# jkaardal/pyipm

Hardware: AMD Instinct MI355X
Metric: newton_steps_per_sec (higher is better)
Workload: dtype f64

## Files before the change

### pyipm_amd/csrc/ctx.hpp

```cpp
#pragma once
#include <hip/hip_runtime.h>
#include <stdint.h>
#include <stdio.h>
#include <stdlib.h>
#include <string.h>
#include <string>
#include <new>
#include <stdexcept>
#include <map>
#include <memory>
#include <vector>
#include "../../include/pyipm_newton.h"
#include "owned.hpp"
#include "step_plan.hpp"

namespace pyipm {

constexpr int TB = PYIPM_TILE;
static_assert(TB == PLAN_TB, "step_plan.hpp states the tile on its own");
constexpr int PADG = PYIPM_PAD;
constexpr int BM = 128;
constexpr int BKU = 16;
constexpr int ROWCHUNK = 2048;

// ... 135 lines not shown
    void factor_timed_out() { factored = false; }
    void factor_returned(int rc, bool keep_forward) {
        if (rc) zeros_clean = false;
        forward_pending = (rc == 0 || rc == PYIPM_E_NONFINITE) && keep_forward && forward_fused;
    }
    void solved(bool direction, bool ray_survives) {
        ev_solve_valid = true; have_direction = direction;
        if (!ray_survives) ray_valid = false;
    }
    void ray_formed() { ray_valid = true; }
    void ray_dropped() { ray_valid = false; }
    void rc_warm_cold() { rc_warm_valid[0] = rc_warm_valid[1] = false; }
    void rc_warm_kept(int phase, bool good) { rc_warm_valid[phase] = good; }
    void storage_handed_out() { zeros_clean = false; storage_exported = true; px_valid = false; }
    void keep_zeros_set() { zeros_clean = false; storage_exported = false; }
    void quiesced() { factored = false; forward_pending = false; forward_fused = false; zeros_clean = false; px_valid = false; }
};

constexpr unsigned long long POLL_TIMEOUT = 200000000ull;
struct PollWords {
    DevBuf<unsigned> buf;
    size_t words; const char* message;
    bool used = false;
    PollWords(size_t words_, const char* message_) : words(words_), message(message_) {}
    unsigned* err() const { return buf + words; }
    hipError_t allocate() { return buf.reserve(words + 1); }
    hipError_t ensure(hipStream_t st) {
        if (buf) return hipSuccess;
        const hipError_t e = allocate();
        return e != hipSuccess ? e : clear_err(st);
    }
    hipError_t arm(size_t n, hipStream_t st) { return hipMemsetAsync(buf, 0, n * sizeof(unsigned), st); }
    hipError_t zero_and_wait(size_t n) {
        const hipError_t e = hipMemset(buf, 0, n * sizeof(unsigned));
        return e != hipSuccess ? e : hipDeviceSynchronize();
    }
    hipError_t fetch_err(int* host, hipStream_t st) const { return hipMemcpyAsync(host, err(), sizeof(int), hipMemcpyDeviceToHost, st); }
    hipError_t clear_err(hipStream_t st) { return hipMemsetAsync(err(), 0, sizeof(unsigned), st); }
};

struct DistState;
struct DistDelete { void operator()(DistState*) const; };

struct Ctx {
    Geo g;
    int batch = 1;
    bool batched = false;
    int64_t b_sH = 0, b_sJe = 0, b_sJi = 0;
    double *b_mu = nullptr, *b_delta = nullptr, *b_delta_c = nullptr, *b_in = nullptr, *b_alpha = nullptr;
    int *b_act = nullptr, *b_in_act = nullptr;
    DevBuf<double> b_merit_buf;
    DevBuf<double> b_solve_buf;
    DevBuf<int> b_form;
    bool b_any_cond = false;
    int device = 0;
    hipStream_t stream = nullptr;
    Stream side;
    Event ev_head, ev_panel, ev_fwd;
    Stream fwd;
    std::vector<Event> ev_done;
    int fuse_forward = 1;
    int lookahead = 2;
    Event ev_early;
    struct TileList { unsigned* dev = nullptr; unsigned count = 0;
                      Event ready; hipStream_t on = nullptr; bool seen_done = false; };
    struct TlArena { DevBuf<unsigned> dev; PinnedBuf<unsigned> host{hipHostMallocDefault}; size_t used = 0; };
    std::vector<TlArena> tl_arenas;
    std::map<std::vector<int64_t>, TileList> tile_lists;
    int skip_zeros = 1;
    int group = 1;
    bool tail_group_user = false;
    int tail_group = 4;
    GroupSched sched;
    double* Wnext = nullptr;
    int group_chain = 1;
    Stream rest;
    std::vector<Event> ev_band;
    Event ev_join, ev_main, ev_split, ev_sfast;
    int keep_zeros = 1;
    int tile_step = 1;
    int sweep_max_blocks = 0;
    int occ_fwd_sweep = 0, occ_bwd_sweep = 0, occ_fwd_prefix = 0, occ_fwd_range = 0;
    int sweep_persist = 1;
    DevBuf<double> sweep_buf;
    DevBuf<double> ms_buf;
    PollWords sweep_words{3 * 4096,
                          "backward sweep (k_bwd_sweep): a poll timed out in an earlier solve; its result was NaN"};
    int dist_slices = 2;
    double dist_timeout_s = 300.0;
    int dist_comm2 = 0;
    int wide_sub = 256;
    int reserve_cus = 16;
    int64_t persist_rows = 12288;
    int num_cus = 256;
    int bulk_bn = 256;
    unsigned long long* dbg_buf = nullptr;
    int condensed = 0;
    int cond_min_refine = 0;
    Geo gc;
    double cond_sigma_max = 1.0e4;
    int64_t cond_na = 0;
    int *cond_pos = nullptr, *cond_idx = nullptr, *cond_cnt = nullptr;
    DevBuf<int> cond_store;
    DevBuf<double> Jx;
    DevBuf<double> JT; double* WT = nullptr;
    double *vc = nullptr, *vt = nullptr;
    double* fwd_vec = nullptr;
    double t_gram = 0;
    bool provider_only = false;
    int reuse_x = 1;
    DevBuf<double> snap;
    int reuse_lam_e = 1;
    DevBuf<double> snap_e;
    DevBuf<unsigned> diag_tiles;
    std::vector<unsigned> diag_tiles_host; int64_t diag_tiles_n = -1;
    int64_t n_reused = 0, n_recorded = 0;
    int fwd_prefix = 1;
    int fwd_prefix_wgs = 96;
    PollWords fwdp_words{4096 + 8192,
                         "forward sweep over the kept panels (k_fwd_prefix): a poll timed out; the direction was NaN "
                         "(PYIPM_FWD_PREFIX=0 runs it panel by panel)"};
    int fwd_range = 1;
    int fwd_range_wgs = 32;
    int64_t fwd_range_key[8] = {-1, -1, -1, -1, -1, -1, -1, -1}, fwd_range_owned = 0;
    PollWords fwdr_words{4096 + 8192,
                         "forward sweep over the kept slack and lambda_e panels (k_fwd_range): a poll timed out; the direction was NaN "
                         "(PYIPM_FWD_RANGE=0 runs it panel by panel)"};
    int slack_one = 1;
    int last_step_kind = 0;
    DevBuf<char> ws;
    double *A = nullptr, *Wbuf = nullptr, *Lbuf = nullptr, *Dinv = nullptr;
    double *Tsv = nullptr;
    double *Tflag = nullptr;
    double *rhs = nullptr, *v0 = nullptr, *v1 = nullptr, *v2 = nullptr, *partial = nullptr;
    double *v3 = nullptr;
    double *df = nullptr, *ce = nullptr, *ci = nullptr, *s = nullptr, *lda = nullptr;
    DevStats* dstats = nullptr;
    unsigned long long* anorm = nullptr;
    const double *d2L = nullptr, *Je = nullptr, *Ji = nullptr;
    int64_t ld_d2L = 0, ld_Je = 0, ld_Ji = 0;
    int sharded = 0;
    std::unique_ptr<DistState, DistDelete> dist;
    DevBuf<double> stg_d2L, stg_Je, stg_Ji;
    double mu = 0.2, eps = 2.220446049250313e-16;
    double delta = 0.0, delta_c = 0.0;
    Held held;
    DevBuf<double> merit_buf, ray_buf;
    const double* ray_for = nullptr; bool ray_quad_given = false;
    int info_steps = 0, info_converged = 0;
    double info_berr0 = -1.0, info_berr = -1.0;
    int rcond_its[2] = {0, 0};
    DevBuf<double> rc_warm_buf;
    double* rc_warm[2] = {nullptr, nullptr};
    double refine_target = 1.0e-14;
    int refine_max = 8;
    double pivtol_rel = 1e-14;
    bool tile_blocked_user = false;
    int tile_blocked = 1;
    int tile_waves = 8;
    int tile_chain = 1;
    int chain_whole = 1;
    int chain_lds_kb = 100;
    bool chain_lds_set = false;
    int chain_cpy = 5;
    static constexpr int CHAIN_SLOTS = 8, CHAIN_WORDS = 160;
    PollWords chain_words{CHAIN_SLOTS * CHAIN_WORDS,
// ... 81 lines not shown
```

### pyipm_amd/csrc/kernels_solve.hpp

```cpp
#pragma once
#include "ctx.hpp"
#include "fwd_range_plan.hpp"

namespace pyipm {

__global__ void k_fwd_diag(const double* __restrict__ A, int64_t ld, int64_t lc0, int64_t c0,
                           int nbw, double* __restrict__ v, int64_t vstride)
{
    extern __shared__ double y[];
    const int tid = threadIdx.x;
    v += (int64_t)blockIdx.y * vstride;
    y[tid] = v[c0 + tid];
    const int nt = nbw / TB;
    for (int u = 0; u + 1 < nt; ++u) {
        __syncthreads();
        if (tid >= (u + 1) * TB) {
            const double* col = A + (c0 + tid) + (lc0 + (int64_t)u * TB) * ld;
            double acc = 0.0;
            #pragma unroll 8
            for (int k = 0; k < TB; ++k) acc = fma(col[(int64_t)k * ld], y[u * TB + k], acc);
            y[tid] -= acc;
        }
    }
    __syncthreads();
    v[c0 + tid] = y[tid];
}

__global__ __launch_bounds__(256) void k_fwd_gemv(const double* __restrict__ A, int64_t ld, int64_t lc0,
                                                  int64_t c0, int nbw, int64_t row_begin, int64_t Npad,
                                                  double* __restrict__ v, int64_t vstride,
                                                  int64_t a0, int64_t a1, int64_t b0, int64_t b1)
{
    extern __shared__ double y[];
    {
        const int64_t i0 = row_begin + (int64_t)blockIdx.x * 256, i1 = i0 + 256;
        if (!((i1 > a0 && i0 < a1) || (i1 > b0 && i0 < b1))) return;
    }
    v += (int64_t)blockIdx.y * vstride;
    for (int k = threadIdx.x; k < nbw; k += 256) y[k] = v[c0 + k];
    __syncthreads();
    const int64_t i = row_begin + (int64_t)blockIdx.x * 256 + threadIdx.x;
    if (i >= Npad) return;
    const double* row = A + i + lc0 * ld;
    double acc0 = 0.0, acc1 = 0.0, acc2 = 0.0, acc3 = 0.0;
    #pragma unroll 4
    for (int k = 0; k < nbw; k += 4) {
        acc0 = fma(row[(int64_t)(k + 0) * ld], y[k + 0], acc0);
        acc1 = fma(row[(int64_t)(k + 1) * ld], y[k + 1], acc1);
        acc2 = fma(row[(int64_t)(k + 2) * ld], y[k + 2], acc2);
        acc3 = fma(row[(int64_t)(k + 3) * ld], y[k + 3], acc3);
    }
    v[i] -= (acc0 + acc1) + (acc2 + acc3);
}

__global__ __launch_bounds__(64) void k_diag_apply(const double* __restrict__ Dinv, const double* __restrict__ Tsave,
                                                   const double* __restrict__ Tflag, int nref, int64_t tile0,
                                                   int64_t c0, double* __restrict__ v, int64_t vstride)
{
    __shared__ double y[TB];
    __shared__ double w[TB];
    const int lane = threadIdx.x;
    v += (int64_t)blockIdx.y * vstride;
    const int64_t base = c0 + (int64_t)blockIdx.x * TB;
    const double y0 = v[base + lane];
    y[lane] = y0;
    __syncthreads();
    const double* X = Dinv + (tile0 + blockIdx.x) * (int64_t)(TB * TB);
    const double* T = Tsave + (tile0 + blockIdx.x) * (int64_t)(TB * TB);
    double z = 0.0;
    #pragma unroll 8
    for (int j = 0; j < TB; ++j) z = fma(X[j * TB + lane], y[j], z);
    if (Tflag[tile0 + blockIdx.x] == 0.0) nref = 0;
    for (int it = 0; it < nref; ++it) {
        w[lane] = z;
        __syncthreads();
        double r = y0;
        #pragma unroll 8
        for (int j = 0; j < TB; ++j) r = fma(-T[j * TB + lane], w[j], r);
        __syncthreads();
        w[lane] = r;
        __syncthreads();
        #pragma unroll 8
        for (int j = 0; j < TB; ++j) z = fma(X[j * TB + lane], w[j], z);
        __syncthreads();
    }
// ... 75 lines not shown
    v[c0 + tid] = x[tid];
}

__global__ __launch_bounds__(1024) void k_bwd_diag4(const double* __restrict__ A, int64_t ld, int64_t lc0, int64_t c0,
                                                    int nbw, int nb, const double* __restrict__ part, int nchunk,
                                                    double* __restrict__ v, int64_t vstride, int64_t pstride)
{
    __shared__ double Ls[3][TB][TB + 1];
    __shared__ double x[4 * TB], ps[4][4 * TB];
    const int tid = threadIdx.x, k = tid & 255, q = tid >> 8;
    v += (int64_t)blockIdx.y * vstride;
    part += (int64_t)blockIdx.y * pstride;
    const int nt = nbw / TB;
    double lt[6][4];
    {
        int idx = 0;
        #pragma unroll
        for (int u = 1; u <= 3; ++u)
            #pragma unroll
            for (int t = 0; t < u; ++t, ++idx)
                #pragma unroll
                for (int r = 0; r < 4; ++r) {
                    const int e = tid + 1024 * r;
                    lt[idx][r] = (u < nt) ? A[(c0 + (int64_t)u * TB + (e & 63)) + (lc0 + t * TB + (e >> 6)) * ld] : 0.0;
                }
    }
    {
        double t = 0.0;
        if (k < nbw) for (int c = q; c < nchunk; c += 4) t += part[(int64_t)c * nb + k];
        ps[q][k] = t;
    }
    __syncthreads();
    if (tid < nbw) x[tid] = v[c0 + tid] - ((ps[0][tid] + ps[1][tid]) + (ps[2][tid] + ps[3][tid]));
    #pragma unroll
    for (int u = 3; u >= 1; --u) {
        if (u < nt) {
            const int base = u * (u - 1) / 2;
            #pragma unroll
            for (int t = 0; t < 3; ++t)
                if (t < u) {
                    #pragma unroll
                    for (int r = 0; r < 4; ++r) { const int e = tid + 1024 * r; Ls[t][e & 63][e >> 6] = lt[base + t][r]; }
                }
            __syncthreads();
            double acc = 0.0;
            if (k < u * TB) {
                const int t = k >> 6, j = k & 63;
                #pragma unroll
                for (int i = 0; i < 16; ++i) acc = fma(Ls[t][16 * q + i][j], x[u * TB + 16 * q + i], acc);
            }
            ps[q][k] = acc;
            __syncthreads();
            if (tid < u * TB) x[tid] -= (ps[0][tid] + ps[1][tid]) + (ps[2][tid] + ps[3][tid]);
        }
    }
    __syncthreads();
    if (tid < nbw) v[c0 + tid] = x[tid];
}


struct SweepGeo {
    int64_t Npad, ld, n, mi, me;
    int nb, npanels, skip;
};
__device__ __forceinline__ double ld_agent(const double* p) { return __hip_atomic_load(p, __ATOMIC_RELAXED, __HIP_MEMORY_SCOPE_AGENT); }
__device__ __forceinline__ void st_agent(double* p, double v) { __hip_atomic_store(p, v, __ATOMIC_RELAXED, __HIP_MEMORY_SCOPE_AGENT); }
__device__ __forceinline__ bool sweep_active(const SweepGeo& sg, int64_t cA, int64_t cB, int64_t r0, int64_t r1) {
    if (!sg.skip || sg.mi == 0) return true;
    const int64_t s0 = sg.n, s1 = sg.n + sg.mi, i0 = sg.n + sg.mi + sg.me;
    if (cB <= s0) return (r0 < s0) || (r1 > s1);
    if (cA >= s0 && cB <= s1) return r1 > i0 + (cA - s0) && r0 < i0 + (cB - s0);
    return true;
}
__device__ __forceinline__ bool sweep_wait(const unsigned* p, unsigned want, unsigned* err, unsigned long long timeout) {
    if (__hip_atomic_load(p, __ATOMIC_RELAXED, __HIP_MEMORY_SCOPE_AGENT) >= want) return true;
    const unsigned long long t0 = wall_clock64();
    for (;;) {
        if (__hip_atomic_load(p, __ATOMIC_RELAXED, __HIP_MEMORY_SCOPE_AGENT) >= want) return true;
        if (__hip_atomic_load(err, __ATOMIC_RELAXED, __HIP_MEMORY_SCOPE_AGENT) != 0u) return false;
        if ((unsigned long long)wall_clock64() - t0 > timeout) { __hip_atomic_store(err, 1u, __ATOMIC_RELAXED, __HIP_MEMORY_SCOPE_AGENT); return false; }
    }
}

__global__ __launch_bounds__(1024) void k_bwd_sweep(const double* __restrict__ A, SweepGeo sg, double* v, unsigned* sync,
                                                    unsigned* err, unsigned long long timeout,
                                                    double* nearbuf,
                                                    unsigned long long* dbg)
{
    __shared__ double Ls[3][TB][TB + 1];
    __shared__ double x[4 * TB], ps[4][4 * TB];
    __shared__ int ok_s;
    const int tid = threadIdx.x, lane = tid & 63, wave = tid >> 6;
    const int P = sg.npanels, nb = sg.nb;
    unsigned* flag = sync; unsigned* nearc = sync + P; unsigned* prog = sync + 2 * P;
    const int gpp = nb / 8;
    if (blockIdx.x == 0) {
        const int k = tid & 255, q = tid >> 8;
        if (tid == 0) ok_s = 1;
        __syncthreads();
        for (int s = P - 1; s >= 0; --s) {
            const int64_t c0 = (int64_t)s * nb;
            int64_t w64 = sg.Npad - c0; if (w64 > nb) w64 = nb;
            const int nbw = (int)w64, nt = nbw / TB;
            double lt[6][4];
            {
                int idx = 0;
                #pragma unroll
                for (int u = 1; u <= 3; ++u)
                    #pragma unroll
                    for (int t = 0; t < u; ++t, ++idx)
                        #pragma unroll
                        for (int r = 0; r < 4; ++r) {
                            const int e = tid + 1024 * r;
                            lt[idx][r] = (u < nt) ? A[(c0 + (int64_t)u * TB + (e & 63)) + (c0 + t * TB + (e >> 6)) * sg.ld] : 0.0;
                        }
            }
            if (dbg && tid == 0) dbg[4 * s + 0] = wall_clock64();
            if (tid < nbw) {
                const double yv = ld_agent(v + c0 + tid);
                double nv = 0.0;
                if (s + 1 < P) {
                    const unsigned long long t0 = wall_clock64();
                    for (;;) {
                        nv = ld_agent(nearbuf + c0 + tid);
                        if (nv == nv) break;
                        if (__hip_atomic_load(nearc + s + 1, __ATOMIC_RELAXED, __HIP_MEMORY_SCOPE_AGENT) >= (unsigned)gpp) { nv = ld_agent(nearbuf + c0 + tid); break; }
                        if (__hip_atomic_load(err, __ATOMIC_RELAXED, __HIP_MEMORY_SCOPE_AGENT) != 0u) { ok_s = 0; break; }
                        if ((unsigned long long)wall_clock64() - t0 > timeout) { __hip_atomic_store(err, 1u, __ATOMIC_RELAXED, __HIP_MEMORY_SCOPE_AGENT); ok_s = 0; break; }
                    }
                }
                x[tid] = yv - nv;
            }
            __syncthreads();
            if (!ok_s) break;
            if (dbg && tid == 0) dbg[4 * s + 1] = wall_clock64();
            #pragma unroll
            for (int u = 3; u >= 1; --u) {
                if (u < nt) {
                    const int base = u * (u - 1) / 2;
                    #pragma unroll
                    for (int t = 0; t < 3; ++t)
                        if (t < u) {
                            #pragma unroll
                            for (int r = 0; r < 4; ++r) { const int e = tid + 1024 * r; Ls[t][e & 63][e >> 6] = lt[base + t][r]; }
                        }
                    __syncthreads();
                    double acc = 0.0;
                    if (k < u * TB) {
                        const int t = k >> 6, j = k & 63;
                        #pragma unroll
                        for (int i = 0; i < 16; ++i) acc = fma(Ls[t][16 * q + i][j], x[u * TB + 16 * q + i], acc);
                    }
                    ps[q][k] = acc;
                    __syncthreads();
                    if (tid < u * TB) x[tid] -= (ps[0][tid] + ps[1][tid]) + (ps[2][tid] + ps[3][tid]);
                }
            }
            __syncthreads();
            if (dbg && tid == 0) dbg[4 * s + 2] = wall_clock64();
            if (tid < nbw) st_agent(v + c0 + tid, x[tid]);
            asm volatile("s_waitcnt vmcnt(0)" ::: "memory");
            __syncthreads();
            if (dbg && tid == 0) dbg[4 * s + 3] = wall_clock64();
            if (tid == 0) __hip_atomic_store(flag + s, 1u, __ATOMIC_RELAXED, __HIP_MEMORY_SCOPE_AGENT);
            if (s + 1 < P && s >= 1 && tid < gpp) {
                const int nwv_o = ((int)gridDim.x - 1 - (gpp + 15) / 16) * 16;
                if (!sweep_wait(prog + ((s - 1) * gpp + tid) % nwv_o, (unsigned)(P - (s + 1)), err, timeout)) ok_s = 0;
            }
            __syncthreads();
            if (!ok_s) break;
        }
        __syncthreads();
        if (__hip_atomic_load(err, __ATOMIC_RELAXED, __HIP_MEMORY_SCOPE_AGENT) != 0u)
            for (int64_t i = tid; i < sg.Npad; i += 1024) st_agent(v + i, __builtin_nan(""));
        return;
    }
    const int nearb_ = (gpp + 15) / 16;
    const bool specialist_ = (int)blockIdx.x <= nearb_;
    const int gw_ = ((int)blockIdx.x - 1 - nearb_) * 16 + wave;
    auto publish = [&](unsigned steps_done) {
        if (lane == 0 && !specialist_) __hip_atomic_store(prog + gw_, steps_done, __ATOMIC_RELAXED, __HIP_MEMORY_SCOPE_AGENT);
    };
    const int nearb = (gpp + 15) / 16;
    const bool specialist = (int)blockIdx.x <= nearb;
    const int nwv = specialist ? 1 : ((int)gridDim.x - 1 - nearb) * 16;
    const int gw = specialist ? ((int)blockIdx.x - 1) * 16 + wave : ((int)blockIdx.x - 1 - nearb) * 16 + wave;
    if (specialist) {
        publish((unsigned)P);
        if (gw >= gpp) return;
    }
    typedef double d2_t __attribute__((ext_vector_type(2)));
    for (int t = P - 1; t >= 1; --t) {
        const int64_t r0 = (int64_t)t * nb;
        int64_t w64 = sg.Npad - r0; if (w64 > nb) w64 = nb;
        const int nbw = (int)w64;
        const int glim = t * gpp;
        if (!specialist && gw >= glim - gpp) break;
        int kmax = specialist ? 0 : (glim - gpp - 1 - gw) / nwv;
        const bool in_rows = 4 * lane < nbw;
        bool have_x = false;
        double xr[4] = {0.0, 0.0, 0.0, 0.0};
        for (int kk = kmax; kk >= 0; --kk) {
            const int g = specialist ? glim - gpp + gw : gw + kk * nwv;
            const int64_t j0 = (int64_t)g * 8;
            const int64_t cp = (j0 / nb) * nb;
            const bool nearg = specialist;
            const bool act = sweep_active(sg, cp, cp + nb, r0, r0 + nbw);
            d2_t la[8][2];
            if (act) {
                #pragma unroll
                for (int c = 0; c < 8; ++c) {
                    if (in_rows) {
                        const double* src = A + (r0 + 4 * lane) + (j0 + c) * sg.ld;
                        la[c][0] = *reinterpret_cast<const d2_t*>(src);
                        la[c][1] = *reinterpret_cast<const d2_t*>(src + 2);
                    } else { la[c][0] = d2_t{0.0, 0.0}; la[c][1] = d2_t{0.0, 0.0}; }
                }
            }
            if (!have_x) {
                if (!sweep_wait(flag + t, 1u, err, timeout)) { publish((unsigned)P); return; }
                asm volatile("" ::: "memory");
                if (in_rows) {
                    const d2_t x01 = *reinterpret_cast<const d2_t*>(v + r0 + 4 * lane), x23 = *reinterpret_cast<const d2_t*>(v + r0 + 4 * lane + 2);
                    xr[0] = x01.x; xr[1] = x01.y; xr[2] = x23.x; xr[3] = x23.y;
                }
                have_x = true;
            }
            if (act) {
                double a[8];
                #pragma unroll
                for (int c = 0; c < 8; ++c)
                    a[c] = fma(la[c][1].y, xr[3], fma(la[c][1].x, xr[2], fma(la[c][0].y, xr[1], la[c][0].x * xr[0])));
                double b4[4], b2[2];
                const bool h5 = (lane & 32) != 0, h4 = (lane & 16) != 0, h3 = (lane & 8) != 0;
                #pragma unroll
                for (int i = 0; i < 4; ++i) {
                    const double send = h5 ? a[i] : a[i + 4], keep = h5 ? a[i + 4] : a[i];
                    b4[i] = keep + __shfl_xor(send, 32, 64);
                }
                #pragma unroll
                for (int i = 0; i < 2; ++i) {
                    const double send = h4 ? b4[i] : b4[i + 2], keep = h4 ? b4[i + 2] : b4[i];
                    b2[i] = keep + __shfl_xor(send, 16, 64);
                }
                double r;
                { const double send = h3 ? b2[0] : b2[1], keep = h3 ? b2[1] : b2[0]; r = keep + __shfl_xor(send, 8, 64); }
                r += __shfl_xor(r, 4, 64); r += __shfl_xor(r, 2, 64); r += __shfl_xor(r, 1, 64);
                if ((lane & 7) == 0) {
                    const int c = (h5 ? 4 : 0) + (h4 ? 2 : 0) + (h3 ? 1 : 0);
                    if (nearg) st_agent(nearbuf + j0 + c, r);
                    else { double* yp = v + j0 + c; st_agent(yp, ld_agent(yp) - r); }
                }
                asm volatile("s_waitcnt vmcnt(0)" ::: "memory");
            } else if (nearg && lane < 8) {
                st_agent(nearbuf + j0 + lane, 0.0);
                asm volatile("s_waitcnt vmcnt(0)" ::: "memory");
            }
            if (nearg && lane == 0) __hip_atomic_fetch_add(nearc + t, 1u, __ATOMIC_RELAXED, __HIP_MEMORY_SCOPE_AGENT);
        }
        if (!specialist) publish((unsigned)(P - t));
    }
    if (!specialist) publish((unsigned)P);
}

__global__ __launch_bounds__(512, 4) void k_fwd_sweep(const double* __restrict__ A, SweepGeo sg, double* v, unsigned* sync,
                                                      unsigned* err, unsigned long long timeout)
{
    __shared__ double xs[4 * TB];
    __shared__ double ps[8][TB];
    __shared__ int ok_s;
    const int tid = threadIdx.x, lane = tid & 63, wave = __builtin_amdgcn_readfirstlane(tid >> 6);
    const int P = sg.npanels, nb = sg.nb;
    unsigned* flag = sync; unsigned* prog = sync + P;
    const int cpp = nb / TB;
    const int nchunks = (int)(sg.Npad / TB);
    if (tid == 0) ok_s = 1;
    __syncthreads();
    if (blockIdx.x == 0) {
        for (int s = 0; s < P; ++s) {
            const int64_t c0 = (int64_t)s * nb;
            int64_t w64 = sg.Npad - c0; if (w64 > nb) w64 = nb;
            const int nbw = (int)w64, nt = nbw / TB;
            double lt[6][8];
            {
                int idx = 0;
                #pragma unroll
                for (int u = 1; u <= 3; ++u)
                    #pragma unroll
                    for (int t = 0; t < u; ++t, ++idx)
                        #pragma unroll
                        for (int r = 0; r < 8; ++r)
                            lt[idx][r] = (u < nt) ? A[(c0 + (int64_t)u * TB + lane) + (c0 + t * TB + wave + 8 * r) * sg.ld] : 0.0;
            }
            if (s > 0 && tid < nt && !sweep_wait(prog + (int)(c0 / TB) + tid, (unsigned)s, err, timeout)) ok_s = 0;
            __syncthreads();
            if (!ok_s) break;
            if (tid < nbw) xs[tid] = ld_agent(v + c0 + tid);
            __syncthreads();
            #pragma unroll
            for (int u = 1; u <= 3; ++u) {
                if (u < nt) {
                    const int base = u * (u - 1) / 2;
                    double acc = 0.0;
                    #pragma unroll
                    for (int t = 0; t < 3; ++t)
                        if (t < u) {
                            #pragma unroll
                            for (int r = 0; r < 8; ++r) acc = fma(lt[base + t][r], xs[t * TB + wave + 8 * r], acc);
                        }
                    ps[wave][lane] = acc;
                    __syncthreads();
                    if (tid < TB) {
                        double t8 = ((ps[0][tid] + ps[1][tid]) + (ps[2][tid] + ps[3][tid])) + ((ps[4][tid] + ps[5][tid]) + (ps[6][tid] + ps[7][tid]));
                        xs[u * TB + tid] -= t8;
                    }
                    __syncthreads();
                }
            }
            if (tid < nbw) st_agent(v + c0 + tid, xs[tid]);
            asm volatile("s_waitcnt vmcnt(0)" ::: "memory");
            __syncthreads();
            if (tid == 0) __hip_atomic_store(flag + s, 1u, __ATOMIC_RELAXED, __HIP_MEMORY_SCOPE_AGENT);
        }
        __syncthreads();
        if (__hip_atomic_load(err, __ATOMIC_RELAXED, __HIP_MEMORY_SCOPE_AGENT) != 0u)
            for (int64_t i = tid; i < sg.Npad; i += 512) st_agent(v + i, __builtin_nan(""));
        return;
    }
    const int nown = (int)gridDim.x - 1;
    for (int s = 0; s + 1 < P; ++s) {
        const int64_t c0 = (int64_t)s * nb;
        const int cfirst = (s + 1) * cpp;
        const int cbeg = cpp + ((int)blockIdx.x - 1);
        int c = cbeg;
        if (c < cfirst) c += ((cfirst - c + nown - 1) / nown) * nown;
        if (c >= nchunks) return;
        const int kc = nb / 8;
        const int64_t jc0 = c0 + (int64_t)wave * kc;
        bool have_y = false;
        for (; c < nchunks; c += nown) {
            const int64_t r0 = (int64_t)c * TB;
            const bool act = sweep_active(sg, c0, c0 + nb, r0, r0 + TB);
            double la[32];
// ... 347 lines not shown
```

### pyipm_amd/csrc/pyipm_newton.hip

```cpp
#include "driver.hpp"
#include "sub_walk.hpp"
#include "kernels_assemble.hpp"
#include "kernels_factor.hpp"
#include "kernels_panel.hpp"
#include "kernels_chain.hpp"
#include "kernels_solve.hpp"
#include "kernels_msolve.hpp"
#include "kernels_batched.hpp"
#include "kernels_merit.hpp"

using namespace pyipm;
using namespace pyipm::drv;

namespace pyipm { namespace drv {


size_t carve_workspace(Ctx* c, const Geo& g, char* base, bool provider_only = false) {
    Carve cv;
    const size_t D = sizeof(double);
    const size_t oA = cv.take(provider_only ? 256 : (size_t)g.Npad * (size_t)(g.ncols_local > 0 ? g.ncols_local : 1) * D);
    const size_t oW = cv.take(provider_only ? 256 : 3 * (size_t)default_group(g.world, g.nb) * (size_t)g.Npad * g.nb * D);
    const size_t oL = cv.take(g.world > 1 ? (size_t)g.Npad * g.nb * D : 256);
    const size_t oD = cv.take(provider_only ? 256 : (size_t)(g.Npad / TB) * TB * TB * D);
    const size_t oT = cv.take(provider_only ? 256 : (size_t)(g.Npad / TB) * TB * TB * D);
// ... 962 lines not shown
int diag_panel(Ctx* ctx, int64_t p, double* v, hipStream_t stream, int nrhs, int64_t vstride) {
    if (!stream) stream = ctx->stream;
    const Geo& g = ctx->g;
    const int64_t c0 = g.panel_c0(p);
    const int nbw = (int)g.panel_w(p);
    hipLaunchKernelGGL(k_diag_apply, dim3(nbw / TB, nrhs), dim3(64), 0, stream, ctx->Dinv, ctx->Tsv, ctx->Tflag, ctx->block_refine,
                       c0 / TB, c0, v, vstride);
    PYIPM_KCHECK();
    return 0;
}

int bwd_panel(Ctx* ctx, int64_t p, double* v, int nrhs, int64_t vstride, double* part, int64_t pstride) {
    const Geo& g = ctx->g;
    if (!part) part = ctx->partial;
    return for_sub_panels(ctx, p, sub_width(ctx, (int)g.panel_w(p)), true, [&](const SweepSub& s) {
        int nchunk = 0;
        if (s.below > 0) {
            nchunk = (int)((s.below + ROWCHUNK - 1) / ROWCHUNK);
            hipLaunchKernelGGL(k_bwd_dot, dim3(s.nbw, nchunk, nrhs), dim3(256), 0, ctx->stream, ctx->A, g.Npad, s.lc0, g.nb,
                               s.c0 + s.nbw, g.Npad, v, part, vstride, pstride, s.a0, s.a1, s.b0, s.b1);
            PYIPM_KCHECK();
        }
        if (s.nbw <= 4 * TB)
            hipLaunchKernelGGL(k_bwd_diag4, dim3(1, nrhs), dim3(1024), 0, ctx->stream, ctx->A, g.Npad, s.lc0, s.c0, s.nbw,
                               g.nb, part, nchunk, v, vstride, pstride);
        else
            hipLaunchKernelGGL(k_bwd_diag, dim3(1, nrhs), dim3(s.nbw), s.nbw * sizeof(double), ctx->stream, ctx->A, g.Npad, s.lc0, s.c0, s.nbw,
                               g.nb, part, nchunk, v, vstride, pstride);
        PYIPM_KCHECK();
        return 0;
    });
}

static bool sweeps_in_one_launch(const Ctx* ctx) {
    const Geo& g = ctx->g;
    return ctx->sweep_persist && g.world == 1 && g.nb <= 4 * TB && g.nb % TB == 0 && g.npanels >= 2 && g.npanels <= 4096 &&
           g.Npad % 8 == 0 && g.Npad / TB <= 8192;
}
static SweepGeo sweep_geo(const Ctx* ctx) {
    const Geo& g = ctx->g;
    SweepGeo sg;
    sg.Npad = g.Npad; sg.ld = g.Npad; sg.n = g.n; sg.mi = g.mi; sg.me = g.me; sg.nb = g.nb; sg.npanels = (int)g.npanels;
    sg.skip = (ctx->skip_zeros && g.mi > 0) ? 1 : 0;
    return sg;
}
template <class K>
static int resident_per_cu(Ctx* ctx, int* occ, K kernel, int threads, const char* must_fit) {
    if (*occ <= 0) PYIPM_HIP(hipOccupancyMaxActiveBlocksPerMultiprocessor(occ, kernel, threads, 0));
    if (*occ < 1 && must_fit) { ctx->err = must_fit; return PYIPM_E_HIP; }
    return 0;
}
static unsigned sweep_grid(const Ctx* ctx, int64_t want, int resident, int64_t floor, int64_t cap = INT64_MAX) {
    int64_t blocks = std::min(std::min(want, (int64_t)resident * ctx->num_cus), cap);
    if (ctx->sweep_max_blocks > 0 && blocks > ctx->sweep_max_blocks) blocks = ctx->sweep_max_blocks;
    return (unsigned)std::max(blocks, floor);
}

static int fwd_sweep(Ctx* ctx, double* v) {
    const Geo& g = ctx->g;
    PollWords& sw = ctx->sweep_words;
    PYIPM_HIP(sw.ensure(ctx->stream));
    PYIPM_HIP(sw.arm((size_t)(g.npanels + g.Npad / TB), ctx->stream));
    { int rc = resident_per_cu(ctx, &ctx->occ_fwd_sweep, k_fwd_sweep, 512, nullptr); if (rc) return rc; }
    const int occ = ctx->occ_fwd_sweep < 1 ? 1 : (ctx->occ_fwd_sweep > 2 ? 2 : ctx->occ_fwd_sweep);
    hipLaunchKernelGGL(k_fwd_sweep, dim3(sweep_grid(ctx, 1 + (g.Npad / TB - g.nb / TB), occ, 2)), dim3(512), 0, ctx->stream,
                       ctx->A, sweep_geo(ctx), v, sw.buf.get(), sw.err(), POLL_TIMEOUT);
    PYIPM_KCHECK();
    hipLaunchKernelGGL(k_diag_apply, dim3((unsigned)(g.Npad / TB), 1), dim3(64), 0, ctx->stream, ctx->Dinv, ctx->Tsv, ctx->Tflag,
                       ctx->block_refine, (int64_t)0, (int64_t)0, v, (int64_t)0);
    PYIPM_KCHECK();
    sw.used = true;
    return 0;
}
static int bwd_sweep(Ctx* ctx, double* v) {
    const Geo& g = ctx->g;
    PollWords& sw = ctx->sweep_words;
    PYIPM_HIP(ctx->sweep_buf.reserve((size_t)g.Npad));
    PYIPM_HIP(sw.ensure(ctx->stream));
    PYIPM_HIP(sw.arm((size_t)(2 * g.npanels + 4096), ctx->stream));
    PYIPM_HIP(hipMemsetAsync(ctx->sweep_buf, 0xFF, (size_t)g.Npad * sizeof(double), ctx->stream));
    const int64_t nearb = (g.nb / 8 + 15) / 16;
    { int rc = resident_per_cu(ctx, &ctx->occ_bwd_sweep, k_bwd_sweep, 1024, "k_bwd_sweep does not fit a compute unit"); if (rc) return rc; }
    const unsigned blocks = sweep_grid(ctx, 1 + nearb + (g.Npad / 8 + 15) / 16, 1, 2 + nearb, 1 + nearb + 4096 / 16);
    hipLaunchKernelGGL(k_bwd_sweep, dim3(blocks), dim3(1024), 0, ctx->stream, ctx->A, sweep_geo(ctx), v, sw.buf.get(), sw.err(),
                       POLL_TIMEOUT, ctx->sweep_buf.get(), ctx->dbg_buf);
    PYIPM_KCHECK();
    sw.used = true;
    return 0;
}

int solve_plain(Ctx* ctx, double* v, bool forward_done, int nrhs, int64_t vstride, double* part, int64_t pstride) {
    const Geo& g = ctx->g;
    const bool one_launch = sweeps_in_one_launch(ctx) && nrhs == 1;
    if (!forward_done && one_launch) {
        int rc = fwd_sweep(ctx, v); if (rc) return rc;
    } else if (!forward_done) {
        for (int64_t p = 0; p < g.npanels; ++p) { int rc = fwd_panel(ctx, p, v, nullptr, nrhs, vstride); if (rc) return rc; }
        for (int64_t p = 0; p < g.npanels; ++p) { int rc = diag_panel(ctx, p, v, nullptr, nrhs, vstride); if (rc) return rc; }
    }
    if (one_launch) return bwd_sweep(ctx, v);
    for (int64_t p = g.npanels - 1; p >= 0; --p) { int rc = bwd_panel(ctx, p, v, nrhs, vstride, part, pstride); if (rc) return rc; }
    return 0;
}

static bool fwd_prefix_applies(const Ctx* ctx) {
    const Geo& g = ctx->g;
    return ctx->fwd_prefix && sweeps_in_one_launch(ctx) && g.nb % (2 * TB) == 0 && sub_width(ctx, (int)g.nb) == (int)g.nb;
}
static int fwd_prefix(Ctx* ctx, int64_t P0, double* v, hipStream_t stream) {
    const Geo& g = ctx->g;
    PollWords& fw = ctx->fwdp_words;
    const int64_t nchunks = g.Npad / TB;
    PYIPM_HIP(fw.ensure(stream));
    PYIPM_HIP(fw.arm((size_t)(P0 + nchunks), stream));
    { int rc = resident_per_cu(ctx, &ctx->occ_fwd_prefix, k_fwd_prefix, 256, "k_fwd_prefix does not fit a compute unit"); if (rc) return rc; }
    const unsigned blocks = sweep_grid(ctx, 1 + (nchunks - g.nb / TB), ctx->occ_fwd_prefix, 2, ctx->fwd_prefix_wgs);
    hipLaunchKernelGGL(k_fwd_prefix, dim3(blocks), dim3(256), 0, stream, ctx->A, sweep_geo(ctx), (int)P0, v, fw.buf.get(), fw.err(),
                       POLL_TIMEOUT);
    PYIPM_KCHECK();
    hipLaunchKernelGGL(k_diag_apply, dim3((unsigned)(P0 * g.nb / TB), 1), dim3(64), 0, stream, ctx->Dinv, ctx->Tsv, ctx->Tflag,
                       ctx->block_refine, (int64_t)0, (int64_t)0, v, (int64_t)0);
    PYIPM_KCHECK();
    fw.used = true;
    return 0;
}

static unsigned fwd_range_grid(Ctx* ctx, int64_t Pa, int64_t Pb) {
    const Geo& g = ctx->g;
    if (!ctx->fwd_range || Pb <= Pa || Pb >= g.npanels) return 0;
    if (resident_per_cu(ctx, &ctx->occ_fwd_range, k_fwd_range, 256, nullptr) || ctx->occ_fwd_range < 1) return 0;
    const SweepGeo sg = sweep_geo(ctx);
    const int64_t key[8] = {sg.Npad, sg.n, sg.mi, sg.me, sg.nb, sg.skip, Pa, Pb};
    if (memcmp(key, ctx->fwd_range_key, sizeof(key)) != 0) {
        const FwdPlanGeo pg{sg.Npad, sg.n, sg.mi, sg.me, sg.nb, sg.skip};
        int64_t owned = 0;
        for (int64_t c = (Pa + 1) * (g.nb / TB); c < g.Npad / TB; ++c) owned += fwd_plan_owned(pg, (int)Pa, (int)Pb, (int)c) ? 1 : 0;
        memcpy(ctx->fwd_range_key, key, sizeof(key)); ctx->fwd_range_owned = owned;
    }
    const int64_t owned = ctx->fwd_range_owned;
    const unsigned blocks = sweep_grid(ctx, 1 + owned, ctx->occ_fwd_range, 2, ctx->fwd_range_wgs);
    return (owned + blocks - 2) / (blocks - 1) <= FWDR_MAXOWN ? blocks : 0;
}
static int fwd_range(Ctx* ctx, int64_t Pa, int64_t Pb, unsigned blocks, double* v, hipStream_t stream) {
    const Geo& g = ctx->g;
    PollWords& fw = ctx->fwdr_words;
    PYIPM_HIP(fw.ensure(stream));
    PYIPM_HIP(fw.arm((size_t)((Pb - Pa) + g.Npad / TB), stream));
    hipLaunchKernelGGL(k_fwd_range, dim3(blocks), dim3(256), 0, stream, ctx->A, sweep_geo(ctx), (int)Pa, (int)Pb, v, fw.buf.get(), fw.err(),
                       POLL_TIMEOUT);
    PYIPM_KCHECK();
    hipLaunchKernelGGL(k_diag_apply, dim3((unsigned)((Pb - Pa) * g.nb / TB), 1), dim3(64), 0, stream, ctx->Dinv, ctx->Tsv, ctx->Tflag,
                       ctx->block_refine, Pa * g.nb / TB, Pa * g.nb, v, (int64_t)0);
    PYIPM_KCHECK();
    fw.used = true;
    return 0;
}

static RowMap all_rows(const Geo& g) { Geo g1 = g; g1.world = 1; g1.rank = 0; return make_rowmap(g1, 0); }

int cond_reduce(Ctx* ctx, const double* b, double* vc) {
    const Geo& g = ctx->g;
    hipLaunchKernelGGL(k_cond_t, grid1(g.mi), dim3(256), 0, ctx->stream, ctx->vt, b, g, ctx->s, ctx->lda + g.me, ctx->eps,
                       ctx->cond_pos);
    PYIPM_KCHECK();
    hipLaunchKernelGGL(k_rowdot2, grid1(g.n, 4), dim3(256), 0, ctx->stream, vc, b, g.n,
                       (const double*)nullptr, (int64_t)0, (const double*)nullptr, (int64_t)0,
                       ctx->Ji, ctx->ld_Ji, ctx->vt, g.mi, 0, 0, all_rows(g));
// ... 765 lines not shown

static int solve_local(Ctx* ctx, const double*, double* x, bool forward_done) { return solve_inplace(ctx, x, forward_done); }
static const SolveOps kLocalOps = {solve_local, kkt_matvec_dev, false};

int assemble_timed(Ctx* ctx, double delta, double delta_c) {
    PYIPM_HIP(hipEventRecord(ctx->ev[2], ctx->stream));
    int rc = assemble_dev(ctx, delta, delta_c); if (rc) return rc;
    PYIPM_HIP(hipEventRecord(ctx->ev[3], ctx->stream));
    ctx->held.assemble_timed();
    return PYIPM_OK;
}

int kkt_matvec_io(Ctx* ctx, const SolveOps& ops, const double* v, double* y, int memkind) {
    const Geo& g = ctx->g;
    ctx->held.borrowed(Held::V1);
    hipLaunchKernelGGL(k_fill, grid1(g.Npad), dim3(256), 0, ctx->stream, ctx->v1, 0.0, g.Npad); PYIPM_KCHECK();
    int rc = put_vec(ctx, ctx->v1, v, g.N, memkind); if (rc) return rc;
    rc = ops.matvec(ctx, ctx->v1, ctx->vc); if (rc) return rc;
    return copy_out(ctx, y, ctx->vc, g.N, memkind);
}

} }

#pragma GCC visibility push(default)
extern "C" {

size_t pyipm_newton_workspace_bytes(int64_t n, int64_t me, int64_t mi, int nb, int world, int rank) try {
    if (n <= 0 || me < 0 || mi < 0 || world < 1 || rank < 0 || rank >= world) return 0;
    if (nb == 0) nb = 256;
    if (nb % 128 != 0 || nb > 1024) return 0;
    Geo g = make_geo(n, me, mi, nb, world, rank);
    return carve_workspace(nullptr, g, nullptr);
} PYIPM_CATCH_SIZE

static int create_handle(pyipm_newton_ctx** out, bool args_ok, int device, void* workspace, size_t workspace_bytes, void* stream,
                         const std::function<void(Ctx*)>& set, const std::function<size_t(Ctx*, char*)>& carve, size_t anorm_words,
                         bool schedule_events) {
    if (!out) return PYIPM_E_BADARG;
    *out = nullptr;
    if (!args_ok) return PYIPM_E_BADARG;
    int ndev = 0;
    if (hipGetDeviceCount(&ndev) != hipSuccess || ndev <= 0 || device < 0 || device >= ndev) return PYIPM_E_NODEVICE;
    std::unique_ptr<Ctx> ctx(new Ctx());
    ctx->device = device;
    ctx->stream = (hipStream_t)stream;
    if (hipSetDevice(device) != hipSuccess) return PYIPM_E_NODEVICE;
    set(ctx.get());
    const size_t need = carve(nullptr, nullptr);
    if (workspace) {
        if (workspace_bytes < need) return PYIPM_E_NOMEM;
        ctx->ws.adopt((char*)workspace, need);
    } else {
        if (ctx->ws.reserve(need) != hipSuccess) return PYIPM_E_NOMEM;
        if (getenv("PYIPM_POISON_WORKSPACE")) hipMemset(ctx->ws, 0xFF, need);
    }
    carve(ctx.get(), ctx->ws.get());
    if (hipMemset(ctx->anorm, 0, anorm_words * sizeof(unsigned long long)) != hipSuccess) return PYIPM_E_HIP;
    for (Event& e : ctx->ev) if (e.ensure(hipEventDefault) != hipSuccess) return PYIPM_E_HIP;
    if (schedule_events) {
        for (Event& e : ctx->ev_prov) if (e.ensure(hipEventDefault) != hipSuccess) return PYIPM_E_HIP;
        for (Event* e : {&ctx->ev_fwd, &ctx->ev_head, &ctx->ev_panel}) if (e->ensure(hipEventDisableTiming) != hipSuccess) return PYIPM_E_HIP;
    }
    *out = reinterpret_cast<pyipm_newton_ctx*>(ctx.release());
    return PYIPM_OK;
}

static int create_impl(pyipm_newton_ctx** out, int64_t n, int64_t me, int64_t mi, int nb, int device,
                       int world, int rank, void* workspace, size_t workspace_bytes, void* stream, bool provider_only) {
    if (nb == 0) nb = 256;
    const bool args_ok = n > 0 && me >= 0 && mi >= 0 && world >= 1 && rank >= 0 && rank < world && nb % 128 == 0 && nb <= 1024;
    const Geo g = args_ok ? make_geo(n, me, mi, nb, world, rank) : Geo{};
    return create_handle(out, args_ok, device, workspace, workspace_bytes, stream,
        [&](Ctx* ctx) {
            ctx->g = g;
            ctx->gc = make_geo(n, me, 0, nb, 1, 0);
            ctx->group = default_group(world, nb);
            { int ncu = 0; if (hipDeviceGetAttribute(&ncu, hipDeviceAttributeMultiprocessorCount, device) == hipSuccess && ncu > 0) ctx->num_cus = ncu; }
            ctx->provider_only = provider_only;
            { const char* e = getenv("PYIPM_REUSE_X"); if (e && e[0] == '0') ctx->reuse_x = 0; }
            { const char* e = getenv("PYIPM_REUSE_LAM_E"); if (e && e[0] == '0') ctx->reuse_lam_e = 0; }
            { const char* e = getenv("PYIPM_FWD_PREFIX"); if (e) { const int w = atoi(e); if (w <= 0) ctx->fwd_prefix = 0; else if (w >= 2) ctx->fwd_prefix_wgs = w; } }
            { const char* e = getenv("PYIPM_FWD_RANGE"); if (e) { const int w = atoi(e); if (w <= 0) ctx->fwd_range = 0; else if (w >= 2) ctx->fwd_range_wgs = w; } }
            { const char* e = getenv("PYIPM_SLACK_ONE"); if (e && atoi(e) <= 0) ctx->slack_one = 0; }
        },
        [&](Ctx* ctx, char* base) { return carve_workspace(ctx, g, base, provider_only); },
        2 , true);
}

int pyipm_newton_create(pyipm_newton_ctx** out, int64_t n, int64_t me, int64_t mi, int nb, int device,
                        int world, int rank, void* workspace, size_t workspace_bytes, void* stream) try {
    return create_impl(out, n, me, mi, nb, device, world, rank, workspace, workspace_bytes, stream, false);
} PYIPM_CATCH_NOH

size_t pyipm_newton_workspace_bytes_provider(int64_t n, int64_t me, int64_t mi) try {
    if (n <= 0 || me < 0 || mi < 0) return 0;
    Geo g = make_geo(n, me, mi, 256, 1, 0);
    return carve_workspace(nullptr, g, nullptr, true);
} PYIPM_CATCH_SIZE

int pyipm_newton_create_provider(pyipm_newton_ctx** out, int64_t n, int64_t me, int64_t mi, int device,
                                 void* workspace, size_t workspace_bytes, void* stream) try {
    return create_impl(out, n, me, mi, 256, device, 1, 0, workspace, workspace_bytes, stream, true);
} PYIPM_CATCH_NOH

size_t pyipm_newton_workspace_bytes_batched(int64_t n, int64_t me, int64_t mi, int batch) try {
    if (n <= 0 || me < 0 || mi < 0 || batch < 1) return 0;
    Geo g = make_geo(n, me, mi, 128, 1, 0);
    if (g.Npad > 1024) return 0;
    return carve_batched(nullptr, g, batch, nullptr);
} PYIPM_CATCH_SIZE

int pyipm_newton_create_batched(pyipm_newton_ctx** out, int64_t n, int64_t me, int64_t mi, int batch, int device,
                                void* workspace, size_t workspace_bytes, void* stream) try {
    bool args_ok = n > 0 && me >= 0 && mi >= 0 && batch >= 1;
    const Geo g = args_ok ? make_geo(n, me, mi, 128, 1, 0) : Geo{};
    args_ok = args_ok && g.Npad <= 1024;
    return create_handle(out, args_ok, device, workspace, workspace_bytes, stream,
        [&](Ctx* ctx) {
            ctx->g = g; ctx->gc = g;
            ctx->batch = batch;
            ctx->group = 1;
            ctx->batched = true;
            ctx->tile_blocked = 1;
        },
        [&](Ctx* ctx, char* base) { return carve_batched(ctx, g, batch, base); },
        (size_t)batch * 2, false);
} PYIPM_CATCH_NOH

static int fetch_batched_stats(Ctx* ctx, pyipm_factor_stats* stats) {
    const int B = ctx->batch;
    std::vector<DevStats> z((size_t)B);
    PYIPM_HIP(hipMemcpyAsync(z.data(), ctx->dstats, (size_t)B * sizeof(DevStats), hipMemcpyDeviceToHost, ctx->stream));
    PYIPM_HIP(hipStreamSynchronize(ctx->stream));
    int rc = PYIPM_OK;
    for (int b = 0; b < B; ++b) {
        stats[b] = to_stats(z[b]);
        if (z[b].nonfinite) { ctx->err = "NaN/Inf met during factorisation"; rc = PYIPM_E_NONFINITE; }
    }
    float ms = 0.f;
    PYIPM_HIP(hipEventElapsedTime(&ms, ctx->ev[0], ctx->ev[1]));
    ctx->t_factor = ms;
    return rc;
}

int pyipm_newton_stage_blocks_batched(pyipm_newton_ctx* h, const double* d2L, int64_t ld_d2L, int64_t stride_d2L,
                                      const double* Je, int64_t ld_Je, int64_t stride_Je,
                                      const double* Ji, int64_t ld_Ji, int64_t stride_Ji) try {
    PYIPM_ENTER("stage_blocks_batched", G_BATCHED) const Geo& g = ctx->g;
    if (!d2L || ld_d2L < g.n || (g.me && (!Je || ld_Je < g.me)) || (g.mi && (!Ji || ld_Ji < g.mi))) {
        ctx->err = "stage_blocks_batched: bad block pointer / leading dimension (device pointers only)"; return PYIPM_E_BADARG; }
    ctx->d2L = d2L; ctx->ld_d2L = ld_d2L; ctx->b_sH = stride_d2L;
    ctx->Je = g.me ? Je : nullptr; ctx->ld_Je = ld_Je; ctx->b_sJe = stride_Je;
    ctx->Ji = g.mi ? Ji : nullptr; ctx->ld_Ji = ld_Ji; ctx->b_sJi = stride_Ji;
    ctx->held.blocks_staged();
    return PYIPM_OK;
} PYIPM_CATCH_H(h)

static int step_batched_enqueue(Ctx* ctx, const BatchEach& in, double* dz, int memkind) {
    const Geo& g = ctx->g;
    const int B = ctx->batch;
    BatchPtrs bp = batch_ptrs(ctx);
    BatchCond bc = batch_cond(ctx);
    const int cond = (ctx->condensed && g.mi > 0) ? 1 : 0;
    ctx->held.step_batched_begun(cond != 0);
    if (ctx->b_form.capacity() < (size_t)B) {
        PYIPM_HIP(ctx->b_form.reserve((size_t)B));
// ... 1082 lines not shown
```

Before: 169.5.

## Skip slack-block panels in backward sweep chain via closed-form pred/succ plan

Adds a backward-chain plan that identifies panels lying entirely in the slack block (columns n..n+mi), whose solution has a closed form, and removes them from the serial diagonal chain of the persistent backward sweep kernel. The diagonal block walks panels via a predecessor function, and the worker waves adjust their progress publication, waits and group ranges so they skip the elided panels. This is meant to shorten the sequential critical path of the backward triangular solve. It adds indexing complexity in the inter-block sync protocol, which risks deadlock or wrong results if the skipped panels are not actually trivial. It can be disabled with an environment variable.

```diff
diff --git a/pyipm_amd/csrc/bwd_chain_plan.hpp b/pyipm_amd/csrc/bwd_chain_plan.hpp
--- /dev/null
+++ b/pyipm_amd/csrc/bwd_chain_plan.hpp
@@ -0,0 +1,25 @@
+#pragma once
+#include <cstdint>
+namespace pyipm {
+struct BwdChainGeo { int64_t Npad, n, mi; int nb, npanels, skip; };
+
+constexpr bool bwd_chain_closed_form(const BwdChainGeo& g, int p) {
+    if (!g.skip || g.mi == 0 || p < 0 || p >= g.npanels) return false;
+    const int64_t c0 = (int64_t)p * g.nb;
+    const int64_t w = g.Npad - c0 < g.nb ? g.Npad - c0 : (int64_t)g.nb;
+    return c0 >= g.n && c0 + w <= g.n + g.mi;
+}
+struct BwdChain { int sa, sb, npanels; };
+constexpr BwdChain bwd_chain(const BwdChainGeo& g, int slack_walk) {
+    const int64_t sa = (g.n + g.nb - 1) / g.nb, sb = (g.n + g.mi) / g.nb;
+    if (!slack_walk || !g.skip || g.mi == 0 || sb <= sa || sb >= g.npanels) return BwdChain{g.npanels, g.npanels, g.npanels};
+    return BwdChain{(int)sa, (int)sb, g.npanels};
+}
+constexpr bool bwd_chain_skipped(const BwdChain& ch, int p) { return p >= ch.sa && p < ch.sb; }
+constexpr int bwd_chain_pred(const BwdChain& ch, int t) { return bwd_chain_skipped(ch, t - 1) ? ch.sa - 1 : t - 1; }
+constexpr int bwd_chain_succ(const BwdChain& ch, int q) { return bwd_chain_skipped(ch, q + 1) ? ch.sb : q + 1; }
+constexpr int bwd_chain_step(const BwdChain& ch, int t) { return ch.npanels - 1 - t - (t < ch.sa ? ch.sb - ch.sa : 0); }
+constexpr int bwd_chain_steps(const BwdChain& ch) { return ch.npanels - (ch.sb - ch.sa); }
+constexpr unsigned bwd_chain_published(const BwdChain& ch, int t) { return (unsigned)(bwd_chain_step(ch, t) + 1); }
+constexpr unsigned bwd_chain_awaited(const BwdChain& ch, int t) { return (unsigned)bwd_chain_step(ch, t); }
+}
diff --git a/pyipm_amd/csrc/ctx.hpp b/pyipm_amd/csrc/ctx.hpp
--- a/pyipm_amd/csrc/ctx.hpp
+++ b/pyipm_amd/csrc/ctx.hpp
@@ -241,6 +241,7 @@
     int sweep_max_blocks = 0;
     int occ_fwd_sweep = 0, occ_bwd_sweep = 0, occ_fwd_prefix = 0, occ_fwd_range = 0;
     int sweep_persist = 1;
+    int bwd_slack = 1;
     DevBuf<double> sweep_buf;
     DevBuf<double> ms_buf;
     PollWords sweep_words{3 * 4096,
diff --git a/pyipm_amd/csrc/kernels_solve.hpp b/pyipm_amd/csrc/kernels_solve.hpp
--- a/pyipm_amd/csrc/kernels_solve.hpp
+++ b/pyipm_amd/csrc/kernels_solve.hpp
@@ -1,6 +1,7 @@
 #pragma once
 #include "ctx.hpp"
 #include "fwd_range_plan.hpp"
+#include "bwd_chain_plan.hpp"
 
 namespace pyipm {
 
@@ -242,7 +243,7 @@
     }
 }
 
-__global__ __launch_bounds__(1024) void k_bwd_sweep(const double* __restrict__ A, SweepGeo sg, double* v, unsigned* sync,
+__global__ __launch_bounds__(1024) void k_bwd_sweep(const double* __restrict__ A, SweepGeo sg, BwdChain ch, double* v, unsigned* sync,
                                                     unsigned* err, unsigned long long timeout,
                                                     double* nearbuf,
                                                     unsigned long long* dbg)
@@ -258,10 +259,11 @@
         const int k = tid & 255, q = tid >> 8;
         if (tid == 0) ok_s = 1;
         __syncthreads();
-        for (int s = P - 1; s >= 0; --s) {
+        for (int s = P - 1, up = P; s >= 0; up = s, s = bwd_chain_pred(ch, s)) {
             const int64_t c0 = (int64_t)s * nb;
             int64_t w64 = sg.Npad - c0; if (w64 > nb) w64 = nb;
             const int nbw = (int)w64, nt = nbw / TB;
+            const int nxt = bwd_chain_pred(ch, s);
             double lt[6][4];
             {
                 int idx = 0;
@@ -279,12 +281,12 @@
             if (tid < nbw) {
                 const double yv = ld_agent(v + c0 + tid);
                 double nv = 0.0;
-                if (s + 1 < P) {
+                if (up < P) {
                     const unsigned long long t0 = wall_clock64();
                     for (;;) {
                         nv = ld_agent(nearbuf + c0 + tid);
                         if (nv == nv) break;
-                        if (__hip_atomic_load(nearc + s + 1, __ATOMIC_RELAXED, __HIP_MEMORY_SCOPE_AGENT) >= (unsigned)gpp) { nv = ld_agent(nearbuf + c0 + tid); break; }
+                        if (__hip_atomic_load(nearc + up, __ATOMIC_RELAXED, __HIP_MEMORY_SCOPE_AGENT) >= (unsigned)gpp) { nv = ld_agent(nearbuf + c0 + tid); break; }
                         if (__hip_atomic_load(err, __ATOMIC_RELAXED, __HIP_MEMORY_SCOPE_AGENT) != 0u) { ok_s = 0; break; }
                         if ((unsigned long long)wall_clock64() - t0 > timeout) { __hip_atomic_store(err, 1u, __ATOMIC_RELAXED, __HIP_MEMORY_SCOPE_AGENT); ok_s = 0; break; }
                     }
@@ -323,9 +325,9 @@
             __syncthreads();
             if (dbg && tid == 0) dbg[4 * s + 3] = wall_clock64();
             if (tid == 0) __hip_atomic_store(flag + s, 1u, __ATOMIC_RELAXED, __HIP_MEMORY_SCOPE_AGENT);
-            if (s + 1 < P && s >= 1 && tid < gpp) {
+            if (up < P && nxt >= 0 && tid < gpp) {
                 const int nwv_o = ((int)gridDim.x - 1 - (gpp + 15) / 16) * 16;
-                if (!sweep_wait(prog + ((s - 1) * gpp + tid) % nwv_o, (unsigned)(P - (s + 1)), err, timeout)) ok_s = 0;
+                if (!sweep_wait(prog + (nxt * gpp + tid) % nwv_o, bwd_chain_awaited(ch, s), err, timeout)) ok_s = 0;
             }
             __syncthreads();
             if (!ok_s) break;
@@ -350,18 +352,21 @@
         if (gw >= gpp) return;
     }
     typedef double d2_t __attribute__((ext_vector_type(2)));
-    for (int t = P - 1; t >= 1; --t) {
+    for (int t = P - 1, q; (q = bwd_chain_pred(ch, t)) >= 0; t = q) {
         const int64_t r0 = (int64_t)t * nb;
         int64_t w64 = sg.Npad - r0; if (w64 > nb) w64 = nb;
         const int nbw = (int)w64;
         const int glim = t * gpp;
-        if (!specialist && gw >= glim - gpp) break;
-        int kmax = specialist ? 0 : (glim - gpp - 1 - gw) / nwv;
+        const int nlo = q * gpp, nhi = nlo + gpp;
+        const int top = nhi == glim ? nlo : glim;
+        if (!specialist && gw >= top) break;
+        int kmax = specialist ? 0 : (top - 1 - gw) / nwv;
         const bool in_rows = 4 * lane < nbw;
         bool have_x = false;
         double xr[4] = {0.0, 0.0, 0.0, 0.0};
         for (int kk = kmax; kk >= 0; --kk) {
-            const int g = specialist ? glim - gpp + gw : gw + kk * nwv;
+            const int g = specialist ? nlo + gw : gw + kk * nwv;
+            if (!specialist && g >= nlo && g < nhi) continue;
             const int64_t j0 = (int64_t)g * 8;
             const int64_t cp = (j0 / nb) * nb;
             const bool nearg = specialist;
@@ -418,7 +423,7 @@
             }
             if (nearg && lane == 0) __hip_atomic_fetch_add(nearc + t, 1u, __ATOMIC_RELAXED, __HIP_MEMORY_SCOPE_AGENT);
         }
-        if (!specialist) publish((unsigned)(P - t));
+        if (!specialist) publish(bwd_chain_published(ch, t));
     }
     if (!specialist) publish((unsigned)P);
 }
diff --git a/pyipm_amd/csrc/pyipm_newton.hip b/pyipm_amd/csrc/pyipm_newton.hip
--- a/pyipm_amd/csrc/pyipm_newton.hip
+++ b/pyipm_amd/csrc/pyipm_newton.hip
@@ -1068,7 +1068,9 @@
     const int64_t nearb = (g.nb / 8 + 15) / 16;
     { int rc = resident_per_cu(ctx, &ctx->occ_bwd_sweep, k_bwd_sweep, 1024, "k_bwd_sweep does not fit a compute unit"); if (rc) return rc; }
     const unsigned blocks = sweep_grid(ctx, 1 + nearb + (g.Npad / 8 + 15) / 16, 1, 2 + nearb, 1 + nearb + 4096 / 16);
-    hipLaunchKernelGGL(k_bwd_sweep, dim3(blocks), dim3(1024), 0, ctx->stream, ctx->A, sweep_geo(ctx), v, sw.buf.get(), sw.err(),
+    const SweepGeo sg = sweep_geo(ctx);
+    const BwdChain ch = bwd_chain(BwdChainGeo{sg.Npad, sg.n, sg.mi, sg.nb, sg.npanels, sg.skip}, ctx->bwd_slack);
+    hipLaunchKernelGGL(k_bwd_sweep, dim3(blocks), dim3(1024), 0, ctx->stream, ctx->A, sg, ch, v, sw.buf.get(), sw.err(),
                        POLL_TIMEOUT, ctx->sweep_buf.get(), ctx->dbg_buf);
     PYIPM_KCHECK();
     sw.used = true;
@@ -2000,6 +2002,7 @@
             { const char* e = getenv("PYIPM_FWD_PREFIX"); if (e) { const int w = atoi(e); if (w <= 0) ctx->fwd_prefix = 0; else if (w >= 2) ctx->fwd_prefix_wgs = w; } }
             { const char* e = getenv("PYIPM_FWD_RANGE"); if (e) { const int w = atoi(e); if (w <= 0) ctx->fwd_range = 0; else if (w >= 2) ctx->fwd_range_wgs = w; } }
             { const char* e = getenv("PYIPM_SLACK_ONE"); if (e && atoi(e) <= 0) ctx->slack_one = 0; }
+            { const char* e = getenv("PYIPM_BWD_SLACK"); if (e && e[0] == '0') ctx->bwd_slack = 0; }
         },
         [&](Ctx* ctx, char* base) { return carve_workspace(ctx, g, base, provider_only); },
         2 , true);
```

New measurement: 175.3, median of 6. 3.4% higher.
